# bytedance/DeepSolid

Hardware: AMD Instinct MI355X
Metric: local-energy evals/sec (higher is better)
Workload: dtype f64; 1 GPU; bcc_li 24 e- (12,12), total_energy primal (E_kin forward-Laplacian + Ewald), default detnet ((256,32),)*3, 8 dets; batch_per_gpu=4096, global_batch=4096, parallelism=walker-dp1

## Files before the change

### deepsolid_amd/_lib.py

```python
import ctypes as C
import os

_HERE = os.path.dirname(os.path.abspath(__file__))
LIB_PATH = os.environ.get('DEEPSOLID_HIP_LIB') or os.path.join(_HERE, 'libdeepsolid_hip.so')

DS_MAX_LAYERS = 8
DS_MAX_SYM = 6
_PD = C.POINTER(C.c_double)


class SystemDesc(C.Structure):
    _fields_ = [
        ('dtype', C.c_int32), ('n_up', C.c_int32), ('n_dn', C.c_int32), ('n_atoms_prim', C.c_int32),
        ('prim_atoms', _PD), ('prim_a', C.c_double * 9), ('sim_a', C.c_double * 9), ('n_sym', C.c_int32),
        ('prim_AV', C.c_double * (DS_MAX_SYM * 3)), ('prim_BV', C.c_double * (DS_MAX_SYM * 3)),
        ('sim_AV', C.c_double * (DS_MAX_SYM * 3)), ('sim_BV', C.c_double * (DS_MAX_SYM * 3)),
        ('n_layers', C.c_int32), ('hidden_single', C.c_int32 * DS_MAX_LAYERS),
        ('hidden_double', C.c_int32 * DS_MAX_LAYERS), ('n_det', C.c_int32), ('distance_type', C.c_int32),
        ('envelope_type', C.c_int32), ('full_det', C.c_int32), ('use_last_layer', C.c_int32),
        ('bias_orbitals', C.c_int32), ('klist_up', _PD), ('klist_dn', _PD),
        ('n_atoms_sim', C.c_int32), ('sim_atoms', _PD), ('sim_charges', _PD), ('dist_mode', C.c_int32),
        ('n_g', C.c_int32), ('gpoints', _PD), ('gweight', _PD), ('ion_exp_re', _PD), ('ion_exp_im', _PD),
        ('ewald_alpha', C.c_double), ('ee_const', C.c_double), ('ei_const', C.c_double), ('ii_total', C.c_double),
    ]
# ... 25 lines not shown
        ('a', C.c_double * 9), ('n_atoms', C.c_int32), ('atoms', _PD), ('atom_species', _PI), ('n_species', C.c_int32),
        ('n_l', _PI), ('r_cut_loc', _PD), ('r_cut_nl', _PD), ('term_offset', _PI), ('term_n', _PI), ('term_zeta', _PD),
        ('term_c', _PD), ('n_quad', C.c_int32),
    ]


_VP = C.c_void_p


def _dmc_step_sig(n_lead, n_noise, n_out, ecp):
    step = [C.c_int64, C.c_int] + [C.c_double] * 5 + [C.c_int, C.c_int, C.c_uint64, C.c_uint64]
    return (C.c_int, [_VP] * n_lead + step + [_VP] * n_noise + ([C.c_int64] if ecp else []) + [C.c_int] + [_VP] * n_out +
            ([C.POINTER(C.c_int)] if ecp else []) + [_VP, C.c_int64, _VP])


SIGNATURES = {
    'ds_device_widths': (C.c_int, [C.POINTER(C.c_int32), C.POINTER(C.c_int32), C.c_int32, C.c_int32, C.c_int32, C.c_int32,
                                   C.POINTER(C.c_int32), C.POINTER(C.c_int32), C.POINTER(C.c_int32), C.POINTER(C.c_int32)]),
    'ds_system_create': (C.c_int, [C.POINTER(SystemDesc), C.POINTER(_VP)]),
    'ds_system_destroy': (None, [_VP]),
    'ds_last_error': (C.c_char_p, []),
    'ds_param_count': (C.c_int64, [_VP]),
    'ds_int8_layers': (C.c_int, [_VP]),
    'ds_param_layout': (C.c_int, [_VP, C.POINTER(ParamBlock), C.c_int]),
    'ds_workspace_bytes': (C.c_int64, [_VP, C.c_int64]),
    'ds_logpsi': (C.c_int, [_VP, _VP, _VP, C.c_int64, _VP, _VP, _VP, C.c_int64, _VP]),
    'ds_logpsi_grad': (C.c_int, [_VP, _VP, _VP, C.c_int64, _VP, _VP, _VP, _VP, C.c_int64, _VP]),
    'ds_vjp_workspace_bytes': (C.c_int64, [_VP, C.c_int64]),
    'ds_logpsi_vjp': (C.c_int, [_VP, _VP, _VP, C.c_int64, _VP, _VP, _VP, _VP, _VP, C.c_int64, _VP]),
    'ds_pretrain_workspace_bytes': (C.c_int64, [_VP, C.c_int64]),
    'ds_pretrain_loss_vjp': (C.c_int, [_VP, _VP, _VP, C.c_int64, _VP, _VP, _VP, _VP, _VP, C.c_int64, _VP]),
    'ds_kfac_block_count': (C.c_int, [_VP]),
    'ds_kfac_layout': (C.c_int, [_VP, C.POINTER(KfacBlock), C.c_int]),
    'ds_kfac_workspace_bytes': (C.c_int64, [_VP, C.c_int64]),
    'ds_kfac_factors': (C.c_int, [_VP, _VP, _VP, C.c_int64, _VP, _VP, _VP, C.c_int64, _VP]),
    'ds_kfac_step_workspace_bytes': (C.c_int64, [_VP]),
    'ds_kfac_inverses': (C.c_int, [_VP, _VP, C.c_double, C.c_double, _VP, _VP, C.c_int64, _VP]),
    'ds_kfac_precondition': (C.c_int, [_VP, _VP, _VP, _VP, _VP, _VP, C.c_int64, _VP]),
    'ds_kfac_inverses_sized_workspace_bytes': (C.c_int64, [C.c_int, C.POINTER(C.c_int32), C.POINTER(C.c_int32)]),
    'ds_kfac_inverses_sized': (C.c_int, [C.c_int, C.c_int, C.POINTER(C.c_int32), C.POINTER(C.c_int32), C.POINTER(C.c_int32), _VP,
                                        C.c_double, C.c_double, _VP, _VP, C.c_int64, _VP]),
    'ds_jacobian_workspace_bytes': (C.c_int64, [_VP, C.c_int64]),
    'ds_logpsi_jacobian': (C.c_int, [_VP, _VP, _VP, C.c_int64, _VP, C.c_int64, _VP, _VP, _VP, C.c_int64, _VP]),
    'ds_minsr_gram_workspace_bytes': (C.c_int64, [C.c_int64, C.c_int64]),
    'ds_minsr_gram': (C.c_int, [C.c_int, _VP, C.c_int64, C.c_int64, C.c_int64, _VP, _VP, C.c_int64, _VP]),
    'ds_minsr_matvec_workspace_bytes': (C.c_int64, [C.c_int, C.c_int64, C.c_int64]),
# ... 96 lines not shown
```

### deepsolid_amd/csrc/ds_api.hip

```cpp
#include <cstdarg>

#include "ds_host.h"
#include "ds_tiles.h"

namespace ds {
#define DS_DECL(p) const TileOps<double>* tile_ops_f64_p##p(int); const TileOps<float>* tile_ops_f32_p##p(int);
DS_DECL(0) DS_DECL(1) DS_DECL(2) DS_DECL(3) DS_DECL(4)
#undef DS_DECL
template <> const TileOps<double>* tile_ops<double>(int st) {
    const TileOps<double>* (*parts[])(int) = {tile_ops_f64_p0, tile_ops_f64_p1, tile_ops_f64_p2, tile_ops_f64_p3, tile_ops_f64_p4};
    for (auto f : parts)
        if (const TileOps<double>* o = f(st)) return o;
    return nullptr;
}
template <> const TileOps<float>* tile_ops<float>(int st) {
    const TileOps<float>* (*parts[])(int) = {tile_ops_f32_p0, tile_ops_f32_p1, tile_ops_f32_p2, tile_ops_f32_p3, tile_ops_f32_p4};
    for (auto f : parts)
        if (const TileOps<float>* o = f(st)) return o;
    return nullptr;
}
}

namespace ds {
namespace host {
// ... 318 lines not shown
        for (int l = 0; l <= s->sd.n_layers; ++l) h1max = std::max(h1max, s->sd.h1[l]);
        if (hipMalloc(&s->lr_w0t, (size_t)h1max * 64 * sizeof(double)) != hipSuccess) {
            ds_system_destroy(s);
            return fail("hipMalloc of the low-rank layer's weight table failed");
        }
    }
    {
        hipDeviceProp_t prop;
        int devid = 0;
        if (hipGetDevice(&devid) == hipSuccess && hipGetDeviceProperties(&prop, devid) == hipSuccess && prop.multiProcessorCount > 0)
            s->n_cu = prop.multiProcessorCount;
    }
    if (hipMalloc((void**)&s->clk_dev, 1024 * sizeof(unsigned long long)) != hipSuccess ||
        hipMemset(s->clk_dev, 0, 1024 * sizeof(unsigned long long)) != hipSuccess) {
        ds_system_destroy(s);
        return fail("hipMalloc of the clock-probe counters failed");
    }
    s->det_valu = getenv("DS_DET_VALU") != nullptr;
    if (const char* e = getenv("DS_VAL_NB")) { const int v = atoi(e); s->val_nb = (v == 1 || v == 2 || v == 4) ? v : 0; }
    s->no_lu_wave = getenv("DS_NO_LU_WAVE") != nullptr;
    s->use_lr = getenv("DS_NO_LOWRANK") == nullptr;
    s->use_pm_skip = getenv("DS_NO_PM_SKIP") == nullptr;
    s->use_pair_expand = getenv("DS_NO_PAIR_EXPAND") == nullptr;
    s->use_g4 = getenv("DS_NO_G4") == nullptr;
    s->use_i8 = getenv("DS_I8") != nullptr && getenv("DS_NO_I8") == nullptr;
    s->use_ldsb = getenv("DS_NO_LDSB") == nullptr;
    s->use_pair_fuse = getenv("DS_NO_PAIR_FUSE") == nullptr;
    s->use_i8_val = getenv("DS_NO_I8_VAL") == nullptr;
    for (int l = 0; l < DS_MAX_LAYERS; ++l) s->i8_prepped[l] = ~(uint64_t)0;
    if (const char* e = getenv("DS_I8_VAL_MIN_TILES")) s->val_i8_min_tiles = atoll(e);
    if (const char* e = getenv("DS_DBG")) s->dbg = atoi(e);
    s->use_wide = getenv("DS_NO_WIDE") == nullptr;
    s->wide_all = getenv("DS_WIDE_ALL") != nullptr;
    {
        const size_t bytes = i8_planes_bytes(s);
        if (bytes && hipMalloc(&s->i8_wp, bytes) != hipSuccess) {
            ds_system_destroy(s);
            return fail("hipMalloc of the int8 layer's weight planes failed");
        }
    }
    if (const char* e = getenv("DS_CHUNK_WALKERS")) s->chunk_cap = std::min<int64_t>(65535, std::max<int64_t>(1, atol(e)));
    *out = s;
    return 0;
}

void ds_system_destroy(ds_system* s) {
// ... 110 lines not shown
```

### deepsolid_amd/csrc/ds_chain.hip

```cpp
#include "ds_host.h"
#include "ds_tiles.h"

namespace ds {
namespace host {

template <typename T> inline unsigned m2_split(int K2, int N) {
    unsigned z = 1;
    while (z < 8 && K2 % (2 * z) == 0 && (size_t)(K2 / z) * 5 * N * sizeof(T) > 8192) z *= 2;
    return z;
}

enum Stop { STOP_NONE = 0, STOP_G0, STOP_G1, STOP_G2, STOP_G3, STOP_H2_0, STOP_H2_1, STOP_H2_2, STOP_MEAN0, STOP_Q,
            STOP_MOUT, STOP_MINV, STOP_DETS, STOP_TR };

template <typename T> struct DumpReq { int stop; T* out; int64_t cap; int64_t written; };

template <typename T>
int copy_out(DumpReq<T>* dr, const T* src, size_t n, hipStream_t st) {
    size_t m = std::min<size_t>(n, (size_t)dr->cap);
    HIP_OK(hipMemcpyAsync(dr->out, src, m * sizeof(T), hipMemcpyDeviceToDevice, st));
    dr->written = (int64_t)m;
    return 0;
}

enum class LayerKind {
    Dense,
    DenseRes,
    L0Stats,
    L0Epi9Means,
    LowRank1,
    Int8
};
struct PairPlan {
    bool res, res_sep;
    bool expand;
    bool write_out;
    unsigned xz; int EW, NW; size_t xlds;
};
struct LayerPlan {
    LayerKind kind;
    bool res_sep;
    bool wide;
    bool pm_mask;
    bool pm_unwritten;
    int prof_kind;
    PairPlan pair;
};
enum class OrbKind { Orb3, Wide, Ldsb, Gemm };
template <typename T> struct ChainPlan {
    const ds::TileOps<T>* to;
    bool lr_on;
    int lr_nc;
    int g4;
    LayerPlan layer[DS_MAX_LAYERS];
    OrbKind orb[2];
    int count(LayerKind k, int n_layers) const {
        int n = 0;
        for (int l = 0; l < n_layers; ++l) n += layer[l].kind == k ? 1 : 0;
        return n;
    }
};

template <typename T>
int plan_chain(const ds_system* s, bool dump, ChainPlan<T>* p) {
    const ds::SysDev<double>& S = s->sd;
    const ds::TileOps<T>* to = p->to = ds::tile_ops<T>(S.P / 16);
    if (!to) return fail("no kernel instance for %d slot tiles (N = %d electrons)", S.P / 16, S.N);
    const int ST = to->ST;
    const bool wide = s->use_wide && to->gemm_wide != nullptr;
    auto gemm_wide = [&](int epi) { return wide && (s->wide_all || ds::gemm_wide_faster<T>(epi)); };
    const int K0loc = S.h1[0] + S.nch * S.h2[0], K0sh = S.nch * S.h1[0];
    p->lr_nc = std::max(2, (K0loc + K0sh + 4 + 15) / 16);
    p->lr_on = !dump && s->use_lr && S.n_layers >= 2 && !s->res1[0] && p->lr_nc <= 4 && S.h1[1] % 16 == 0 && (S.nch * S.h2[1]) % 4 == 0 &&
               3 * (K0loc + K0sh + 4) <= S.h1[1] && p->lr_nc * S.h1[1] < (S.h1[1] - K0loc - K0sh - 4) * ST;
    const int used = S.D - 16 * (ST - 1);
    p->g4 = !s->use_g4 ? 0 : (ST == 5 && used > 8 && used <= 12) ? 3 : (ST == 10 && used <= 4) ? 1 : 0;
    for (int l = 0; l < S.n_layers; ++l) {
        const int Kh = S.h1[l], K2 = S.h2[l], Nout = S.h1[l + 1], Kloc = Kh + S.nch * K2;
        LayerPlan& lp = p->layer[l];
        lp = LayerPlan{};
        if (Nout % 64 || Nout > 1024) return fail("hidden_single must be a multiple of 64 and <= 1024 (got %d)", Nout);
        if (l < S.n_double) {
            PairPlan& pp = lp.pair;
            const int K2o = S.h2[l + 1];
            if (K2o != 32 && K2o != 16) return fail("hidden_double must be 16 or 32 (got %d)", K2o);
            if (K2 % 4) return fail("pair-stream width %d is not a multiple of 4", K2);
            pp.res_sep = s->res2[l] && l == 0;
            pp.res = s->res2[l] && !pp.res_sep;
            pp.xz = (!pp.res && K2o == 32) ? 2 : 1;
            pp.write_out = l + 1 < S.n_double || s->use_last;
            pp.EW = (pp.write_out && S.N % 16 == 8 && pp.xz == 2) ? 2 : 1;
            pp.NW = (pp.EW * S.N + 15) / 16;
            pp.xlds = ((size_t)(K2o / pp.xz) * 5 * pp.EW * S.N + (size_t)pp.EW * S.nch * (K2o / pp.xz) * 5) * sizeof(T);
            pp.expand = !dump && s->use_pair_expand && !pp.res_sep && l + 1 < S.n_layers && pp.NW <= 8 && pp.xlds <= 150 * 1024;
        }
        const bool res = s->res1[l];
        lp.res_sep = res && l == 0 && (Kloc % 16 != 0 || S.nf * S.A != Nout);
        if (res && !lp.res_sep && Kloc % 16) return fail("residual layer with K = %d: the GEMM's operand ring needs K %% 16 == 0", Kloc);
        if (p->lr_on && l == 1) {
            lp.kind = LayerKind::LowRank1;
            lp.wide = wide && (s->wide_all || ds::lr_wide_faster<T>(p->lr_nc));
        } else if (p->lr_on && l == 0) {
            const bool one_kernel = to->layer0_stats && ds::layer0_stats_instance(ST, K0loc / 4);
            lp.kind = one_kernel ? LayerKind::L0Stats : LayerKind::L0Epi9Means;
            lp.wide = !one_kernel && gemm_wide(9);
        } else if (int8_energy_layer(s, l)) {
            lp.kind = LayerKind::Int8;
        } else if (res && !lp.res_sep) {
            lp.kind = LayerKind::DenseRes;
            lp.wide = gemm_wide(2);
        } else {
            lp.kind = LayerKind::Dense;
            lp.wide = gemm_wide(1);
        }
        lp.prof_kind = l == 0 ? DS_PROF_SINGLE_FIRST : (lp.kind == LayerKind::LowRank1 ? DS_PROF_SINGLE_LR : DS_PROF_SINGLE_HIDDEN);
        lp.pm_mask = s->use_pm_skip && (l == 0 || (lp.kind == LayerKind::DenseRes && Kh % 16 == 0 && K2 % 16 == 0));
        lp.pm_unwritten = !dump && l >= 1 && !lp.wide &&
// ... 39 lines not shown
    }
    if (stop == STOP_MEAN0) return copy_out(dr, c.MEAN[0], (size_t)S.nch * S.h1[0] * S.P * Bc, st);
    if (stop == STOP_H2_0) return copy_out(dr, c.H2[0], (size_t)S.h2[0] * 5 * S.NP * Bc, st);
    if (stop == STOP_Q) return copy_out(dr, c.Q, L.Q * Bc, st);
    int gi = 0, hi = 0;
    for (int l = 0; l < S.n_layers; ++l) {
        const LayerPlan& lp = plan.layer[l];
        const int Kh = S.h1[l], K2 = S.h2[l], Nout = S.h1[l + 1];
        if (!(l > 0 && plan.layer[l - 1].pair.expand)) {
            ProfScope ps(s, DS_PROF_M2_EXPAND, st);
            const bool xl = lr_on && l == 0;
            hipLaunchKernelGGL((ds::k_m2_expand<T>), dim3(S.N, (unsigned)Bc, m2_split<T>(K2, S.N)), dim3(256), (size_t)(K2 * 5 * S.N + S.nch * K2 * 5) / m2_split<T>(K2, S.N) * sizeof(T), st, S,
                               c.H2[hi], K2, xl ? c.XL : c.G[gi], Kh, xl ? K0loc : S.ldk, lp.pm_unwritten ? 1 : 0);
        }
        if (stop == STOP_G0 + l) return copy_out(dr, c.G[gi], L.G * Bc, st);
        if (l < S.n_double) {
            const PairPlan& pp = lp.pair;
            const int K2o = S.h2[l + 1];
            const T* W2 = blk(s->i_w2[l]); const T* b2 = blk(s->i_b2[l]);
            ProfScope ps(s, DS_PROF_TWO_LAYER, st);
            if (pp.expand) {
#define DS_TWOX(NT2, RES) hipLaunchKernelGGL((ds::k_two_layer_expand<T, NT2, RES>), dim3(S.N / pp.EW, (unsigned)Bc, pp.xz), dim3(64 * pp.NW), pp.xlds, st, S, c.H2[hi], K2, W2, b2, \
                                             pp.write_out ? c.H2[hi ^ 1] : (T*)nullptr, c.G[gi ^ 1], S.h1[l + 1], S.ldk, plan.layer[l + 1].pm_unwritten ? 1 : 0, pp.EW)
                if (K2o == 32 && pp.res) DS_TWOX(2, true);
                else if (pp.res) DS_TWOX(1, true);
                else DS_TWOX(1, false);
#undef DS_TWOX
            } else {
                const dim3 grid((S.NP / 16 + 3) / 4, (unsigned)Bc);
#define DS_TWO(NT2, RES) hipLaunchKernelGGL((ds::k_two_layer<T, NT2, RES, false>), grid, dim3(256), 0, st, S, c.H2[hi], K2, W2, b2, c.H2[hi ^ 1])
                if (K2o == 32) { if (pp.res) DS_TWO(2, true); else DS_TWO(2, false); }
                else { if (pp.res) DS_TWO(1, true); else DS_TWO(1, false); }
#undef DS_TWO
            }
            if (pp.res_sep)
                launch_pair_res_add<T>(dim3((unsigned)(((size_t)K2o * 5 * S.NP + 255) / 256), (unsigned)Bc), st, c.H2[hi], K2, c.H2[hi ^ 1], K2o, S.nf, S.NP);
        }
        const int Kloc = Kh + S.nch * K2, Ksh = S.nch * Kh;
        {
            dim3 block; unsigned gz;
            gemm_geom(Nout, NB, &block, &gz, ST);
            dim3 wblock; unsigned wgz;
            gemm_geom(Nout, 4, &wblock, &wgz, 6);
            const size_t gws = (size_t)S.N * S.ldk * S.P, gts = (size_t)S.ldk * S.P;
            const bool lr1 = lp.kind == LayerKind::LowRank1;
            T* Sl = lr1 ? c.ZB + (size_t)Bc * S.h1[1] * S.P : c.ZB;
            {
                ProfScope ps(s, DS_PROF_SHARED_TERM, st);
                if (l == 0 || lr1) {
// ... 39 lines not shown
                                   (size_t)S.N * K0loc * S.P, (size_t)K0loc * S.P, blk(s->i_wloc[0]), K0loc, c.ZB, Nout, S.P, c.YO, c.MEAN[1]);
                break;
            }
            case LayerKind::Int8: {
                launch_layer_i8(s, l, false, (const double*)blk(s->i_wloc[l]), Kloc, Nout, (const double*)c.G[gi], gts, (const double*)Sl,
                                (double*)c.G[gi ^ 1], (int)(Bc * S.N), st);
                break;
            }
            case LayerKind::DenseRes:
                ga.oe.dbg = s->dbg & 3;
                ga.oe.g4 = plan.g4;
                if (l > 0 && s->prof_on && (s->prof_only < 0 || s->prof_only == DS_PROF_SINGLE_HIDDEN)) { ga.oe.clk = s->clk_dev; ga.oe.dbg = s->dbg; }
                layer_gemm(2, ga);
                break;
            case LayerKind::Dense:
                layer_gemm(1, ga);
                if (lp.res_sep)
                    launch_layer_res_add<T>(dim3(S.N, (unsigned)Bc), st, Xin, xws, xts, c.G[gi ^ 1], gws, gts, S.nf * S.A, Nout, S.P);
                break;
            }
        }
        gi ^= 1;
        if (l < S.n_double) {
            hi ^= 1;
            if (stop == STOP_H2_1 + l) return copy_out(dr, c.H2[hi], (size_t)S.h2[l + 1] * 5 * S.NP * Bc, st);
        }
    }
    if (stop == STOP_G0 + S.n_layers) return copy_out(dr, c.G[gi], L.G * Bc, st);
    const int Kl = S.h1[S.n_layers], K2l = S.h2[S.n_layers];
    if (s->use_last) {
        ProfScope ps(s, DS_PROF_M2_EXPAND, st);
        hipLaunchKernelGGL((ds::k_m2_expand<T>), dim3(S.N, (unsigned)Bc, m2_split<T>(K2l, S.N)), dim3(256), (size_t)(K2l * 5 * S.N + S.nch * K2l * 5) / m2_split<T>(K2l, S.N) * sizeof(T), st, S,
                           c.H2[hi], K2l, c.G[gi], Kl, S.ldk, 0);
    }
    for (int sp = 0; sp < S.nch; ++sp) {
        const int ns = sp == 0 ? S.n_up : S.n_dn, i0 = sp == 0 ? 0 : S.n_up, OC = S.ocols[sp];
        const int Korb = Kl + (s->use_last ? S.nch * K2l : 0);
        dim3 block; unsigned gz;
        gemm_geom(OC, NB, &block, &gz, ST);
        if (s->use_last) {
            ProfScope ps(s, DS_PROF_SHARED_TERM, st);
            to->shared_term(dim3(1, (unsigned)Bc, gz), block, 2 * 16 * S.P * sizeof(T), st, S, c.G[gi], blk(s->i_wsh_orb[sp]), Kl, c.ZB, OC, S.P,
                            (const T*)nullptr, 0);
        }
        ProfScope ps(s, DS_PROF_ORBITAL, st);
        const int ch = S.mat_ch[sp];
        ds::OrbEpi<T> oe{c.Q, c.MOUT, L.MOUT, L.mout_off[ch], S.N, i0, S.nparam[sp], S.nparam_max, S.norb[sp], S.det_n[ch],
// ... 110 lines not shown
    const ds::SysDev<T>& S = dev<T>(s);
    size_t sh = ds::ewald_lds_bytes(S);
    hipLaunchKernelGGL((ds::k_ewald<T>), dim3((unsigned)B), dim3(256), sh, st, S, (const T*)x, (T*)out);
}

template <typename T>
int64_t debug_stage_impl(ds_system* s, const void* params, const void* x, int64_t B, int stop, void* out, int64_t out_elems, void* ws,
                         int64_t ws_bytes, hipStream_t st) {
    DumpReq<T> dr{stop, (T*)out, out_elems, 0};
    const int rc = run_chain<T>(s, (const T*)params, (const T*)x, B, arena_of<T>(ws, ws_bytes), st, nullptr, nullptr, nullptr, &dr);
    return rc ? -1 : dr.written;
}

int logpsi_grad_forward(ds_system* s, const void* params, const void* x, int64_t B, void* out_logabs, void* out_phase, void* out_grad,
                        void* ws, int64_t ws_bytes, hipStream_t st) {
    return DS_BY_DTYPE(s->dtype, logpsi_grad_impl, s, params, x, B, out_logabs, out_phase, out_grad, ws, ws_bytes, st);
}

int int8_energy_layers(const ds_system* s, bool dump) {
    ChainPlan<double> plan;
    return plan_chain<double>(s, dump, &plan) == 0 ? plan.count(LayerKind::Int8, s->sd.n_layers) : 0;
}

template <typename T> void launch_pair_res_add(dim3 grid, hipStream_t st, const T* Hin, int Kin, T* Hout, int Kout, int n_res, int NP) {
    hipLaunchKernelGGL((ds::k_pair_res_add<T>), grid, dim3(256), 0, st, Hin, Kin, Hout, Kout, n_res, NP);
}

template <typename T>
void launch_layer_res_add(dim3 grid, hipStream_t st, const T* Xin, size_t x_ws, size_t x_ts, T* Gout, size_t g_ws, size_t g_ts, int n_res,
                          int Nout, int P) {
    hipLaunchKernelGGL((ds::k_layer_res_add<T>), grid, dim3(256), 0, st, Xin, x_ws, x_ts, Gout, g_ws, g_ts, n_res, Nout, P);
}

#define DS_INST(T)                                                                                      \
    template void launch_pair_res_add<T>(dim3, hipStream_t, const T*, int, T*, int, int, int);          \
    template void launch_layer_res_add<T>(dim3, hipStream_t, const T*, size_t, size_t, T*, size_t, size_t, int, int, int);
DS_INST(double) DS_INST(float)
#undef DS_INST

}
}

using namespace ds::host;

extern "C" {

int ds_int8_layers(const ds_system* s) {
    if (!s) return -1;
    return int8_energy_layers(s, false);
}

int ds_local_energy(ds_system* s, const void* params, const void* x, int64_t B, void* out_ke, void* out_ewald, void* out_logabs,
                    void* out_phase, void* ws, int64_t ws_bytes, void* stream) {
    if (s) ++s->call_seq;
    if (!s || !params || !x || !ws) return fail("null argument");
    if (B <= 0) return 0;
    hipStream_t st = (hipStream_t)stream;
    return DS_BY_DTYPE(s->dtype, local_energy_impl, s, params, x, B, out_ke, out_ewald, out_logabs, out_phase, ws, ws_bytes, st);
}

int ds_logpsi_grad(ds_system* s, const void* params, const void* x, int64_t B, void* out_logabs, void* out_phase, void* out_grad,
                   void* ws, int64_t ws_bytes, void* stream) {
    if (s) ++s->call_seq;
    if (!s || !params || !x || !ws || !out_grad) return fail("null argument");
    if (B <= 0) return 0;
    hipStream_t st = (hipStream_t)stream;
    return logpsi_grad_forward(s, params, x, B, out_logabs, out_phase, out_grad, ws, ws_bytes, st);
}

int ds_ewald(ds_system* s, const void* x, int64_t B, void* out, void* stream) {
    if (!s || !x || !out) return fail("null argument");
    if (B <= 0) return 0;
// ... 27 lines not shown
```

### deepsolid_amd/csrc/ds_host.h

```cpp
#pragma once
#include "ds_base.h"
#include "ds_value.h"

namespace ds {
namespace host {

template <typename I> inline I rup(I x, int m) { return (x + m - 1) / m * m; }

template <typename T> struct Arena {
    T* base = nullptr;
    size_t cap = SIZE_MAX, used = 0;
    bool ok = true;
    T* take(size_t n) { T* p = base ? base + used : nullptr; used += n; ok = ok && used <= cap; return p; }
    void align(size_t k) { take((k - used % k) % k); }
    template <typename F> void part(T* buf, size_t n, F&& carve) { Arena a{buf, n}; carve(a); ok = ok && a.ok; }
};
template <typename T> Arena<T> arena_of(void* ws, int64_t ws_bytes) { return Arena<T>{(T*)ws, (size_t)std::max<int64_t>(ws_bytes, 0) / sizeof(T)}; }
template <typename F> size_t measure(F&& layout) { Arena<double> a; layout(a); return a.used; }

struct PassSize { size_t fixed, per_group; };
inline int64_t groups_per_pass(int64_t B, int64_t esz, const PassSize& z, int64_t budget) {
    const int64_t groups = std::min<int64_t>((std::max<int64_t>(B, 1) + ds::PV - 1) / ds::PV, 64);
    return std::max<int64_t>(1, std::min<int64_t>(groups, budget / ((int64_t)z.per_group * esz)));
}
// ... 16 lines not shown
}

struct ds_system {
    ds_system_desc d;
    int dtype;
    ds::SysDev<double> sd;
    ds::SysDev<float> sf;
    void* blob64 = nullptr;
    void* blob32 = nullptr;
    std::vector<ds_param_block> blocks;
    int64_t nparams = 0;
    ds::host::WsLayout ws;
    ds::host::WsLayout wsv;
    std::vector<int> i_wloc, i_wsh, i_b, i_w2, i_b2, i_worb, i_wsh_orb, i_borb, i_pi, i_sg;
    bool use_last = false;
    int32_t ref_single[DS_MAX_LAYERS] = {0}, ref_double[DS_MAX_LAYERS] = {0};
    bool res1[DS_MAX_LAYERS] = {false}, res2[DS_MAX_LAYERS] = {false};
    bool no_lu_wave = false;
    int val_nb = 0;
    bool det_valu = false;
    int64_t chunk_cap = 4096;
    bool use_g4 = true;
    bool use_pair_expand = true;
    bool use_pm_skip = true;
    bool use_lr = true;
    void* lr_w0t = nullptr;
    int64_t val_i8_min_tiles = 512;
    bool use_i8_val = true;
    bool use_pair_fuse = true;
    bool use_ldsb = true;
    bool use_i8 = false;
    void* i8_wp = nullptr;
    uint64_t call_seq = 0;
    uint64_t i8_prepped[DS_MAX_LAYERS];
    int n_cu = 256;
    bool use_wide = true;
    bool wide_all = false;
    int dbg = 0;
    bool prof_on = false;
    int prof_only = -1;
    std::vector<std::pair<hipEvent_t, hipEvent_t>> prof_ev[DS_PROF_KINDS];
    std::vector<hipEvent_t> prof_pool;
    unsigned long long* clk_dev = nullptr;
    bool prof_failed = false;
};

// ... 175 lines not shown
```

### deepsolid_amd/csrc/ds_kernels.h

```cpp
#pragma once
#include "ds_device.h"

namespace ds {

#define DS_MAXL 8

template <typename T> struct SysDev {
    int N, n_up, n_dn, A, L, K, nch;
    int D, P, NP;
    int n_layers, n_double;
    int h1[DS_MAXL + 1];
    int h2[DS_MAXL + 1];
    int ldk;
    int full_det, env_type, bias_orb;
    int dist_type, nf;
    int norb[2];
    int n_detch;
    int det_n[2];
    int mat_ch[2], row_off[2];
    int nparam[2];
    int nparam_max;
    int ocols[2];
    const T *prim_a, *prim_ainv, *sim_a, *sim_ainv, *prim_AV, *prim_BV, *sim_AV, *sim_BV, *atoms;
    const T* klist[2];
// ... 191 lines not shown
template <typename T>
__global__ void __launch_bounds__(256) k_layer_res_add(const T* __restrict__ Xin, size_t x_ws, size_t x_ts, T* __restrict__ Gout, size_t g_ws,
                                                       size_t g_ts, int n_res, int Nout, int P) {
    const T* xi = Xin + (size_t)blockIdx.y * x_ws + (size_t)blockIdx.x * x_ts;
    T* go = Gout + (size_t)blockIdx.y * g_ws + (size_t)blockIdx.x * g_ts;
    const T rs2 = T(0.70710678118654752440);
    for (int idx = threadIdx.x; idx < Nout * P; idx += blockDim.x) {
        const T r = idx < n_res * P ? xi[idx] : T(0);
        go[idx] = (r + go[idx]) * rs2;
    }
}

template <typename T>
__global__ void __launch_bounds__(256) k_pair_res_add(const T* __restrict__ Hin, int Kin, T* __restrict__ Hout, int Kout, int n_res, int NP) {
    const size_t idx = (size_t)blockIdx.x * blockDim.x + threadIdx.x;
    if (idx >= (size_t)Kout * 5 * NP) return;
    const T* hi = Hin + (size_t)blockIdx.y * Kin * 5 * NP;
    T* ho = Hout + (size_t)blockIdx.y * Kout * 5 * NP;
    const T r = idx < (size_t)n_res * 5 * NP ? hi[idx] : T(0);
    ho[idx] = (r + ho[idx]) * T(0.70710678118654752440);
}

constexpr int PM_SLOTS = 3;
template <typename T, int NT2, bool RES, bool VAL>
__global__ void __launch_bounds__(256, ((RES && !VAL && sizeof(T) == 8 && NT2 == 2) ? 2 : 3)) k_two_layer(SysDev<T> S, const T* __restrict__ Hin, int Kin, const T* __restrict__ W,
                                                   const T* __restrict__ bias, T* __restrict__ Hout, T* __restrict__ PARTM = nullptr) {
    typedef typename Acc4<T>::type acc_t;
    const int w = blockIdx.y, wave = threadIdx.x >> 6, lane = threadIdx.x & 63;
    const int pt = blockIdx.x * 4 + wave, NP = S.NP, Kout = 16 * NT2;
    if (pt * 16 >= NP) return;
    const int lr = lane & 15, lq = lane >> 4;
    const T* Hw = Hin + (size_t)w * Kin * 5 * NP + pt * 16 + lr;
    acc_t acc[NT2][5];
#pragma unroll
    for (int a = 0; a < NT2; ++a)
#pragma unroll
        for (int c = 0; c < 5; ++c) acc[a][c] = acc_t{0, 0, 0, 0};
    constexpr bool KEEP = RES && !VAL && sizeof(T) == 8;
    T bk[KEEP ? 4 * NT2 : 1][5];
    if constexpr (KEEP) {
#pragma unroll
        for (int ks = 0; ks < 4 * NT2; ++ks)
#pragma unroll
            for (int c = 0; c < 5; ++c) bk[ks][c] = Hw[(size_t)((4 * ks + lq) * 5 + c) * NP];
#pragma unroll
        for (int ks = 0; ks < 4 * NT2; ++ks) {
// ... 16 lines not shown
        for (int a = 0; a < NT2; ++a)
#pragma unroll
            for (int c = 0; c < 5; ++c) acc[a][c] = mfma16(av[a], bv[c], acc[a][c]);
    }
    const T rs2 = T(0.70710678118654752440);
    T* Ho = Hout + (size_t)w * Kout * 5 * NP + pt * 16 + lr;
    __shared__ T pm_stage[VAL ? 4 * PM_SLOTS * 16 * NT2 * 5 : 1];
    T* pm_lds = pm_stage + (VAL ? wave * (PM_SLOTS * Kout * 5) : 0);
    bool pm_valid = false, pm_last = false;
    int pm_slot = 0;
    if (VAL && PARTM) {
        const int N = S.N, nch = S.nch;
        auto seg_of = [&](int p) { const int e = p / N, j = p - e * N; return p < N * N ? e * nch + (nch > 1 && j >= S.n_up ? 1 : 0) : -1; };
        const int p = pt * 16 + lr, sg = seg_of(p);
        pm_valid = sg >= 0;
        pm_slot = sg - seg_of(pt * 16);
        pm_last = pm_valid && (lr == 15 || seg_of(p + 1) != sg);
    }
#pragma unroll
    for (int a = 0; a < NT2; ++a)
#pragma unroll
        for (int r = 0; r < 4; ++r) {
            const int n = 16 * a + acc_row<T>(lane, r);
            const T z0 = acc[a][0][r] + bias[n];
            const T y = ds_tanh(z0), d1 = 1 - y * y, d2 = -2 * y * d1;
            const T z1 = acc[a][1][r], z2 = acc[a][2][r], z3 = acc[a][3][r], z4 = acc[a][4][r];
            T o[5] = {y, d1 * z1, d1 * z2, d1 * z3, d1 * z4 + d2 * 2 * (z1 * z1 + z2 * z2 + z3 * z3)};
            if (VAL) {
                o[1] = ds_tanh(z1 + bias[n]); o[2] = ds_tanh(z2 + bias[n]); o[3] = ds_tanh(z3 + bias[n]); o[4] = ds_tanh(z4 + bias[n]);
            }
#pragma unroll
            for (int c = 0; c < 5; ++c) {
                T v = o[c];
                if (RES) v = ((KEEP ? bk[KEEP ? 4 * a + r : 0][c] : Hw[(size_t)(n * 5 + c) * NP]) + v) * rs2;
                if (Hout) Ho[(size_t)(n * 5 + c) * NP] = v;
                if (VAL && PARTM) {
                    const T pre = row16_prefix(pm_valid ? v : T(0));
                    if (pm_last) pm_lds[(pm_slot * Kout + n) * 5 + c] = pre;
                }
            }
        }
    if (VAL && PARTM) {
        __builtin_amdgcn_fence(__ATOMIC_ACQ_REL, "wavefront");
        __builtin_amdgcn_wave_barrier();
        T* pm = PARTM + ((size_t)w * (NP / 16) + pt) * (PM_SLOTS * Kout * 5);
        for (int i = lane; i < PM_SLOTS * Kout * 5; i += 64) pm[i] = pm_lds[i];
    }
}

template <typename T, int NT2, bool RES>
__global__ void __launch_bounds__(512) k_two_layer_expand(SysDev<T> S, const T* __restrict__ Hin, int Kin, const T* __restrict__ W,
                                                          const T* __restrict__ bias, T* __restrict__ Hout, T* __restrict__ G, int row0,
                                                          int ldg, int skip, int EW) {
    typedef typename Acc4<T>::type acc_t;
    extern __shared__ __attribute__((aligned(16))) char smem_raw[];
    const int w = blockIdx.y, wave = threadIdx.x >> 6, lane = threadIdx.x & 63, tid = threadIdx.x, nt = blockDim.x;
    const int N = S.N, NP = S.NP, P = S.P, Kout = 16 * NT2, e0 = blockIdx.x * EW, PW = EW * N;
    const int KT = Kout * gridDim.z, n0 = Kout * blockIdx.z;
    const int lr = lane & 15, lq = lane >> 4;
    const bool valid = wave * 16 + lr < PW;
    const int pl = valid ? wave * 16 + lr : PW - 1;
    const T* Hw = Hin + (size_t)w * Kin * 5 * NP + e0 * N + pl;
    T* hs = reinterpret_cast<T*>(smem_raw);
    T* sums = hs + Kout * 5 * PW;
    acc_t acc[NT2][5];
#pragma unroll
    for (int a = 0; a < NT2; ++a)
#pragma unroll
        for (int c = 0; c < 5; ++c) acc[a][c] = acc_t{0, 0, 0, 0};
    constexpr bool KEEP = RES && sizeof(T) == 8;
    T bk[KEEP ? 4 * NT2 : 1][5];
    if constexpr (KEEP) {
#pragma unroll
        for (int ks = 0; ks < 4 * NT2; ++ks)
#pragma unroll
            for (int c = 0; c < 5; ++c) bk[ks][c] = Hw[(size_t)((4 * ks + lq) * 5 + c) * NP];
#pragma unroll
        for (int ks = 0; ks < 4 * NT2; ++ks) {
            T av[NT2];
#pragma unroll
            for (int a = 0; a < NT2; ++a) av[a] = W[(size_t)(4 * ks + lq) * KT + n0 + 16 * a + lr];
#pragma unroll
            for (int a = 0; a < NT2; ++a)
#pragma unroll
                for (int c = 0; c < 5; ++c) acc[a][c] = mfma16(av[a], bk[ks][c], acc[a][c]);
        }
    } else
    for (int ks = 0; ks < Kin / 4; ++ks) {
        T av[NT2], bv[5];
#pragma unroll
        for (int a = 0; a < NT2; ++a) av[a] = W[(size_t)(4 * ks + lq) * KT + n0 + 16 * a + lr];
#pragma unroll
        for (int c = 0; c < 5; ++c) bv[c] = Hw[(size_t)((4 * ks + lq) * 5 + c) * NP];
#pragma unroll
        for (int a = 0; a < NT2; ++a)
#pragma unroll
            for (int c = 0; c < 5; ++c) acc[a][c] = mfma16(av[a], bv[c], acc[a][c]);
    }
    const T rs2 = T(0.70710678118654752440);
    T* Ho = (Hout && valid) ? Hout + ((size_t)w * KT + n0) * 5 * NP + e0 * N + pl : nullptr;
#pragma unroll
    for (int a = 0; a < NT2; ++a)
#pragma unroll
        for (int r = 0; r < 4; ++r) {
            const int n = 16 * a + acc_row<T>(lane, r);
            const T z0 = acc[a][0][r] + bias[n0 + n];
            const T y = ds_tanh(z0), d1 = 1 - y * y, d2 = -2 * y * d1;
            const T z1 = acc[a][1][r], z2 = acc[a][2][r], z3 = acc[a][3][r], z4 = acc[a][4][r];
            const T o[5] = {y, d1 * z1, d1 * z2, d1 * z3, d1 * z4 + d2 * 2 * (z1 * z1 + z2 * z2 + z3 * z3)};
#pragma unroll
            for (int c = 0; c < 5; ++c) {
                T v = o[c];
                if (RES) v = ((KEEP ? bk[KEEP ? 4 * a + r : 0][c] : Hw[(size_t)((n0 + n) * 5 + c) * NP]) + v) * rs2;
                if (Ho) Ho[(size_t)(n * 5 + c) * NP] = v;
                if (valid) hs[(n * 5 + c) * PW + pl] = v;
            }
        }
    __syncthreads();
    const int nch = S.nch;
    for (int idx = tid; idx < EW * nch * Kout * 5; idx += nt) {
        const int kc = idx % (5 * Kout), es = idx / (5 * Kout), s = es % nch, el = es / nch;
        const int j0 = s == 0 ? 0 : S.n_up, ns = s == 0 ? S.n_up : S.n_dn;
        T v = 0;
        for (int j = j0; j < j0 + ns; ++j) v += hs[kc * PW + el * N + j];
        sums[idx] = v / T(ns);
    }
    __syncthreads();
    typedef T vec4 __attribute__((ext_vector_type(4)));
    const int QP = P / 4;
    for (int idx = tid; idx < EW * nch * Kout * QP; idx += nt) {
        const int row = idx / QP, sq = idx - row * QP, k = row % Kout, es = row / Kout, s = es % nch, el = es / nch, e = e0 + el;
        const int j0 = s == 0 ? 0 : S.n_up, ns = s == 0 ? S.n_up : S.n_dn;
        if (skip) {
            const int t = sq >> 2, lo = (2 + 3 * j0) >> 4, hi = (4 + 3 * (j0 + ns - 1)) >> 4;
            if (!(t == 0 || t == ((2 + 3 * e) >> 4) || t == ((4 + 3 * e) >> 4) || (t >= lo && t <= hi))) continue;
        }
        const T inv = T(1) / T(ns);
        const T* sm = sums + (es * Kout + k) * 5;
        vec4 v;
#pragma unroll
        for (int u = 0; u < 4; ++u) {
            const int slot = 4 * sq + u;
            T x = 0;
            if (slot == 0) x = sm[0];
            else if (slot == 1) x = sm[4];
            else if (slot < S.D) {
                const int j = (slot - 2) / 3, c = (slot - 2) - 3 * j;
                if (j == e) x = -sm[1 + c];
                else if (j >= j0 && j < j0 + ns) x = hs[(k * 5 + 1 + c) * PW + el * N + j] * inv;
            }
            v[u] = x;
        }
        *reinterpret_cast<vec4*>(G + ((size_t)(w * N + e) * ldg + row0 + s * KT + n0 + k) * P + 4 * sq) = v;
    }
}

template <typename T>
__global__ void __launch_bounds__(256) k_m2_combine_val(SysDev<T> S, const T* __restrict__ PARTM, int K2, T* __restrict__ G, int row0, int RC) {
    constexpr int PV_ = 80;
    extern __shared__ __attribute__((aligned(16))) char smem_raw[];
    T* out = reinterpret_cast<T*>(smem_raw);
    const int e = blockIdx.x, g = blockIdx.y, N = S.N, nt = S.NP / 16, nch = S.nch;
    const int r0 = blockIdx.z * RC, sp = r0 / K2, k0 = r0 - sp * K2;
    const size_t blk = (size_t)PM_SLOTS * K2 * 5;
    const int a = e * N + (sp == 0 ? 0 : S.n_up), ns = sp == 0 ? S.n_up : S.n_dn, b = a + ns;
    const int seg = e * nch + sp;
    for (int idx = threadIdx.x; idx < RC * PV_; idx += blockDim.x) {
        const int cc = idx % 5, kk = (idx / 5) % RC, w5 = idx / (5 * RC), k = k0 + kk;
        const T* pw = PARTM + ((size_t)g * (PV_ / 5) + w5) * nt * blk;
        T v = 0;
        for (int pt = a / 16; pt <= (b - 1) / 16; ++pt) {
            const int p0 = pt * 16, e0 = p0 / N, j0 = p0 - e0 * N, seg0 = e0 * nch + (nch > 1 && j0 >= S.n_up ? 1 : 0);
            const int q = seg - seg0;
            v += pw[(size_t)pt * blk + ((size_t)q * K2 + k) * 5 + cc] - (q > 0 ? pw[(size_t)pt * blk + ((size_t)(q - 1) * K2 + k) * 5 + cc] : T(0));
        }
        out[kk * PV_ + w5 * 5 + cc] = v / T(ns);
// ... 950 lines not shown
```

### deepsolid_amd/device.py

```python
import ctypes as C
import re
from typing import NamedTuple

import numpy as np
import torch

from . import _lib
from .params import ParamMap

_DTYPES = {torch.float64: 0, torch.float32: 1}


def _pd(a):
    return a.ctypes.data_as(C.POINTER(C.c_double))


def _ptr(t):
    return C.c_void_p(t.data_ptr()) if t is not None else C.c_void_p(0)


def _stream():
    return C.c_void_p(torch.cuda.current_stream().cuda_stream)


# ... 793 lines not shown
        return dict(e_loc=energy[:, 0], e_nl=torch.complex(energy[:, 1], energy[:, 2]), pairs=pairs if want_pairs else None,
                    rotations=rot, pair_capacity=cap,
                    ratios=torch.view_as_complex(ratios)[:int(pairs.sum()) * ecp.n_quad] if want_ratios else None)

    def energy_stats(self, ke, ew):
        out = torch.empty(8, dtype=torch.float64, device=self.device)
        _lib.check(self.lib.ds_energy_stats(self.handle, _ptr(ke), _ptr(ew), ke.shape[0], _ptr(out), _stream()), 'ds_energy_stats')
        return out

    def profile(self, on=True, only=None):
        mode = 0 if not on else (1 if only is None else 2 + _lib.PROF_KINDS.index(only))
        _lib.check(self.lib.ds_profile_enable(self.handle, mode), 'ds_profile_enable')

    def profile_read(self):
        n = len(_lib.PROF_KINDS)
        ms = (C.c_double * n)()
        cnt = (C.c_int64 * n)()
        _lib.check(self.lib.ds_profile_read(self.handle, ms, cnt), 'ds_profile_read')
        return {k: (float(ms[i]), int(cnt[i])) for i, k in enumerate(_lib.PROF_KINDS)}

    def int8_layers(self):
        return int(self.lib.ds_int8_layers(self.handle))

    def profile_clock(self):
        cyc, ticks = C.c_double(0), C.c_double(0)
        _lib.check(self.lib.ds_profile_read_clock(self.handle, C.byref(cyc), C.byref(ticks)), 'ds_profile_read_clock')
        return cyc.value, ticks.value, (cyc.value / ticks.value * 0.1 if ticks.value > 0 else None)

    def debug_stage(self, params, x, stage, n_elems):
        x = self._check_x(x)
        p = self.pack_params(params)
        ws = self.workspace(x.shape[0])
        out = torch.zeros(int(n_elems), dtype=self.dtype, device=self.device)
        n = self.lib.ds_debug_stage(self.handle, _ptr(p), _ptr(x), x.shape[0], stage.encode(), _ptr(out), out.numel(),
                                    _ptr(ws), ws.numel(), _stream())
        if n < 0:
            raise RuntimeError(f'ds_debug_stage({stage}): {self.lib.ds_last_error().decode()}')
        return out[:n]


def observable_sums(recvec, x, q_int, pol_direction):
    _require_gpu()
    if not x.is_cuda:
        raise RuntimeError('observable_sums: walkers must live on the ROCm device (no CPU path)')
    if x.dtype not in _DTYPES:
        raise TypeError(f'observable_sums: walkers must be float64 or float32, got {x.dtype}')
# ... 238 lines not shown
```

### include/deepsolid_hip.h

```cpp
#ifndef DEEPSOLID_HIP_H
#define DEEPSOLID_HIP_H

#include <stddef.h>
#include <stdint.h>

#ifdef __cplusplus
extern "C" {
#endif

#define DS_MAX_LAYERS 8
#define DS_MAX_SYM 6

typedef struct ds_system ds_system;

typedef struct ds_system_desc {
    int32_t dtype;
    int32_t n_up, n_dn;
    int32_t n_atoms_prim;
    const double* prim_atoms;
    double prim_a[9];
    double sim_a[9];
    int32_t n_sym;
    double prim_AV[DS_MAX_SYM * 3], prim_BV[DS_MAX_SYM * 3];
    double sim_AV[DS_MAX_SYM * 3], sim_BV[DS_MAX_SYM * 3];
// ... 18 lines not shown
    const double* ion_exp_re;
    const double* ion_exp_im;
    double ewald_alpha;
    double ee_const;
    double ei_const;
    double ii_total;
} ds_system_desc;

typedef struct ds_param_block {
    int64_t offset;
    int32_t rows, cols;
} ds_param_block;

int ds_device_widths(const int32_t* hidden_single, const int32_t* hidden_double, int32_t n_layers, int32_t n_in_single,
                     int32_t n_in_double, int32_t n_double, int32_t* dev_single, int32_t* dev_double, int32_t* res_single,
                     int32_t* res_double);

int ds_system_create(const ds_system_desc* desc, ds_system** out);
void ds_system_destroy(ds_system* sys);
const char* ds_last_error(void);

int ds_int8_layers(const ds_system* sys);

int64_t ds_param_count(const ds_system* sys);
int ds_param_layout(const ds_system* sys, ds_param_block* blocks, int max_blocks);

int64_t ds_workspace_bytes(const ds_system* sys, int64_t B);

int ds_logpsi(ds_system* sys, const void* params, const void* x, int64_t B,
              void* out_logabs, void* out_phase, void* ws, int64_t ws_bytes, void* stream);

int ds_logpsi_grad(ds_system* sys, const void* params, const void* x, int64_t B,
                   void* out_logabs, void* out_phase, void* out_grad, void* ws, int64_t ws_bytes, void* stream);

int64_t ds_vjp_workspace_bytes(const ds_system* sys, int64_t B);
int ds_logpsi_vjp(ds_system* sys, const void* params, const void* x, int64_t B, const void* cot, void* grad,
                  void* out_logabs, void* out_phase, void* ws, int64_t ws_bytes, void* stream);

int64_t ds_pretrain_workspace_bytes(const ds_system* sys, int64_t B);
int ds_pretrain_loss_vjp(ds_system* sys, const void* params, const void* x, int64_t B, const void* target_up,
                         const void* target_dn, void* out_loss, void* grad, void* ws, int64_t ws_bytes, void* stream);

typedef struct ds_kfac_block {
    int32_t kind, index;
    int32_t n_param_blocks;
    int32_t param_blocks[3];
// ... 216 lines not shown
```

Before: 67580 local-energy evals/s.

## Recompute narrow preceding pair layer inside residual expand kernel instead of storing it

When a float64 residual pair layer follows a narrow (≤8 wide) non-residual expanded pair layer, the previous layer no longer writes its pair-stream output. The next expand kernel recomputes that layer's tanh jet from its input via MFMA and keeps the result in registers, which removes a global write and read of the pair activations at the cost of redundant matmul work. The G-scatter loop in the expand kernel is also restructured so per-slot indexing is hoisted out of the row loop. A query API reports how many layers use the recompute path, and an env var disables it.

```diff
diff --git a/deepsolid_amd/_lib.py b/deepsolid_amd/_lib.py
--- a/deepsolid_amd/_lib.py
+++ b/deepsolid_amd/_lib.py
@@ -71,6 +71,7 @@
     'ds_last_error': (C.c_char_p, []),
     'ds_param_count': (C.c_int64, [_VP]),
     'ds_int8_layers': (C.c_int, [_VP]),
+    'ds_pair_recompute_layers': (C.c_int, [_VP, C.c_int]),
     'ds_param_layout': (C.c_int, [_VP, C.POINTER(ParamBlock), C.c_int]),
     'ds_workspace_bytes': (C.c_int64, [_VP, C.c_int64]),
     'ds_logpsi': (C.c_int, [_VP, _VP, _VP, C.c_int64, _VP, _VP, _VP, C.c_int64, _VP]),
diff --git a/deepsolid_amd/csrc/ds_api.hip b/deepsolid_amd/csrc/ds_api.hip
--- a/deepsolid_amd/csrc/ds_api.hip
+++ b/deepsolid_amd/csrc/ds_api.hip
@@ -364,6 +364,7 @@
     s->use_lr = getenv("DS_NO_LOWRANK") == nullptr;
     s->use_pm_skip = getenv("DS_NO_PM_SKIP") == nullptr;
     s->use_pair_expand = getenv("DS_NO_PAIR_EXPAND") == nullptr;
+    s->use_pair_recompute = getenv("DS_NO_PAIR_RECOMPUTE") == nullptr;
     s->use_g4 = getenv("DS_NO_G4") == nullptr;
     s->use_i8 = getenv("DS_I8") != nullptr && getenv("DS_NO_I8") == nullptr;
     s->use_ldsb = getenv("DS_NO_LDSB") == nullptr;
diff --git a/deepsolid_amd/csrc/ds_chain.hip b/deepsolid_amd/csrc/ds_chain.hip
--- a/deepsolid_amd/csrc/ds_chain.hip
+++ b/deepsolid_amd/csrc/ds_chain.hip
@@ -36,6 +36,7 @@
     bool expand;
     bool write_out;
     unsigned xz; int EW, NW; size_t xlds;
+    bool recompute_prev;
 };
 struct LayerPlan {
     LayerKind kind;
@@ -75,6 +76,12 @@
                3 * (K0loc + K0sh + 4) <= S.h1[1] && p->lr_nc * S.h1[1] < (S.h1[1] - K0loc - K0sh - 4) * ST;
     const int used = S.D - 16 * (ST - 1);
     p->g4 = !s->use_g4 ? 0 : (ST == 5 && used > 8 && used <= 12) ? 3 : (ST == 10 && used <= 4) ? 1 : 0;
+    auto pair_geom = [&](PairPlan& pp, int K2o) {
+        pp.xz = (!pp.res && K2o == 32) ? 2 : 1;
+        pp.EW = (pp.write_out && S.N % 16 == 8 && pp.xz == 2) ? 2 : 1;
+        pp.NW = (pp.EW * S.N + 15) / 16;
+        pp.xlds = ((size_t)(K2o / pp.xz) * 5 * pp.EW * S.N + (size_t)pp.EW * S.nch * (K2o / pp.xz) * 5) * sizeof(T);
+    };
     for (int l = 0; l < S.n_layers; ++l) {
         const int Kh = S.h1[l], K2 = S.h2[l], Nout = S.h1[l + 1], Kloc = Kh + S.nch * K2;
         LayerPlan& lp = p->layer[l];
@@ -87,12 +94,18 @@
             if (K2 % 4) return fail("pair-stream width %d is not a multiple of 4", K2);
             pp.res_sep = s->res2[l] && l == 0;
             pp.res = s->res2[l] && !pp.res_sep;
-            pp.xz = (!pp.res && K2o == 32) ? 2 : 1;
             pp.write_out = l + 1 < S.n_double || s->use_last;
-            pp.EW = (pp.write_out && S.N % 16 == 8 && pp.xz == 2) ? 2 : 1;
-            pp.NW = (pp.EW * S.N + 15) / 16;
-            pp.xlds = ((size_t)(K2o / pp.xz) * 5 * pp.EW * S.N + (size_t)pp.EW * S.nch * (K2o / pp.xz) * 5) * sizeof(T);
+            pair_geom(pp, K2o);
             pp.expand = !dump && s->use_pair_expand && !pp.res_sep && l + 1 < S.n_layers && pp.NW <= 8 && pp.xlds <= 150 * 1024;
+            if (l >= 1) {
+                PairPlan& prev = p->layer[l - 1].pair;
+                pp.recompute_prev = sizeof(T) == 8 && !dump && s->use_pair_recompute && pp.res && pp.expand && S.h2[l - 1] <= 8 &&
+                                    !prev.res && !prev.res_sep && prev.expand;
+                if (pp.recompute_prev) {
+                    prev.write_out = false;
+                    pair_geom(prev, K2);
+                }
+            }
         }
         const bool res = s->res1[l];
         lp.res_sep = res && l == 0 && (Kloc % 16 != 0 || S.nf * S.A != Nout);
@@ -178,9 +191,15 @@
             if (pp.expand) {
 #define DS_TWOX(NT2, RES) hipLaunchKernelGGL((ds::k_two_layer_expand<T, NT2, RES>), dim3(S.N / pp.EW, (unsigned)Bc, pp.xz), dim3(64 * pp.NW), pp.xlds, st, S, c.H2[hi], K2, W2, b2, \
                                              pp.write_out ? c.H2[hi ^ 1] : (T*)nullptr, c.G[gi ^ 1], S.h1[l + 1], S.ldk, plan.layer[l + 1].pm_unwritten ? 1 : 0, pp.EW)
-                if (K2o == 32 && pp.res) DS_TWOX(2, true);
+#define DS_TWOXP(NT2) hipLaunchKernelGGL((ds::k_two_layer_expand<T, NT2, true, true>), dim3(S.N / pp.EW, (unsigned)Bc, pp.xz), dim3(64 * pp.NW), pp.xlds, st, S, c.H2[hi ^ 1], S.h2[l - 1], W2, b2, \
+                                         pp.write_out ? c.H2[hi] : (T*)nullptr, c.G[gi ^ 1], S.h1[l + 1], S.ldk, plan.layer[l + 1].pm_unwritten ? 1 : 0, pp.EW,               \
+                                         blk(s->i_w2[l - 1]), blk(s->i_b2[l - 1]))
+                if (pp.recompute_prev) {
+                    if constexpr (sizeof(T) == 8) { if (K2o == 32) DS_TWOXP(2); else DS_TWOXP(1); }
+                } else if (K2o == 32 && pp.res) DS_TWOX(2, true);
                 else if (pp.res) DS_TWOX(1, true);
                 else DS_TWOX(1, false);
+#undef DS_TWOXP
 #undef DS_TWOX
             } else {
                 const dim3 grid((S.NP / 16 + 3) / 4, (unsigned)Bc);
@@ -266,7 +285,7 @@
         }
         gi ^= 1;
         if (l < S.n_double) {
-            hi ^= 1;
+            if (!lp.pair.recompute_prev) hi ^= 1;
             if (stop == STOP_H2_1 + l) return copy_out(dr, c.H2[hi], (size_t)S.h2[l + 1] * 5 * S.NP * Bc, st);
         }
     }
@@ -423,6 +442,14 @@
     return plan_chain<double>(s, dump, &plan) == 0 ? plan.count(LayerKind::Int8, s->sd.n_layers) : 0;
 }
 
+template <typename T> int pair_recompute_count(const ds_system* s, bool dump) {
+    ChainPlan<T> plan;
+    if (plan_chain<T>(s, dump, &plan)) return 0;
+    int n = 0;
+    for (int l = 0; l < s->sd.n_double && l < s->sd.n_layers; ++l) n += plan.layer[l].pair.recompute_prev ? 1 : 0;
+    return n;
+}
+
 template <typename T> void launch_pair_res_add(dim3 grid, hipStream_t st, const T* Hin, int Kin, T* Hout, int Kout, int n_res, int NP) {
     hipLaunchKernelGGL((ds::k_pair_res_add<T>), grid, dim3(256), 0, st, Hin, Kin, Hout, Kout, n_res, NP);
 }
@@ -449,6 +476,11 @@
 int ds_int8_layers(const ds_system* s) {
     if (!s) return -1;
     return int8_energy_layers(s, false);
+}
+
+int ds_pair_recompute_layers(const ds_system* s, int dump) {
+    if (!s) return -1;
+    return s->dtype == 0 ? pair_recompute_count<double>(s, dump != 0) : pair_recompute_count<float>(s, dump != 0);
 }
 
 int ds_local_energy(ds_system* s, const void* params, const void* x, int64_t B, void* out_ke, void* out_ewald, void* out_logabs,
diff --git a/deepsolid_amd/csrc/ds_host.h b/deepsolid_amd/csrc/ds_host.h
--- a/deepsolid_amd/csrc/ds_host.h
+++ b/deepsolid_amd/csrc/ds_host.h
@@ -62,6 +62,7 @@
     int64_t chunk_cap = 4096;
     bool use_g4 = true;
     bool use_pair_expand = true;
+    bool use_pair_recompute = true;
     bool use_pm_skip = true;
     bool use_lr = true;
     void* lr_w0t = nullptr;
diff --git a/deepsolid_amd/csrc/ds_kernels.h b/deepsolid_amd/csrc/ds_kernels.h
--- a/deepsolid_amd/csrc/ds_kernels.h
+++ b/deepsolid_amd/csrc/ds_kernels.h
@@ -237,6 +237,13 @@
 }
 
 constexpr int PM_SLOTS = 3;
+template <typename T>
+__device__ __forceinline__ void pair_tanh_jet(T z0, T z1, T z2, T z3, T z4, T (&o)[5]) {
+    const T y = ds_tanh(z0), d1 = 1 - y * y, d2 = -2 * y * d1;
+    o[0] = y; o[1] = d1 * z1; o[2] = d1 * z2; o[3] = d1 * z3;
+    o[4] = d1 * z4 + d2 * 2 * (z1 * z1 + z2 * z2 + z3 * z3);
+}
+__device__ __forceinline__ double as_loaded(double x) { asm("" : "+v"(x)); return x; }
 template <typename T, int NT2, bool RES, bool VAL>
 __global__ void __launch_bounds__(256, ((RES && !VAL && sizeof(T) == 8 && NT2 == 2) ? 2 : 3)) k_two_layer(SysDev<T> S, const T* __restrict__ Hin, int Kin, const T* __restrict__ W,
                                                    const T* __restrict__ bias, T* __restrict__ Hout, T* __restrict__ PARTM = nullptr) {
@@ -299,10 +306,9 @@
 #pragma unroll
         for (int r = 0; r < 4; ++r) {
             const int n = 16 * a + acc_row<T>(lane, r);
-            const T z0 = acc[a][0][r] + bias[n];
-            const T y = ds_tanh(z0), d1 = 1 - y * y, d2 = -2 * y * d1;
             const T z1 = acc[a][1][r], z2 = acc[a][2][r], z3 = acc[a][3][r], z4 = acc[a][4][r];
-            T o[5] = {y, d1 * z1, d1 * z2, d1 * z3, d1 * z4 + d2 * 2 * (z1 * z1 + z2 * z2 + z3 * z3)};
+            T o[5];
+            pair_tanh_jet(acc[a][0][r] + bias[n], z1, z2, z3, z4, o);
             if (VAL) {
                 o[1] = ds_tanh(z1 + bias[n]); o[2] = ds_tanh(z2 + bias[n]); o[3] = ds_tanh(z3 + bias[n]); o[4] = ds_tanh(z4 + bias[n]);
             }
@@ -325,10 +331,11 @@
     }
 }
 
-template <typename T, int NT2, bool RES>
+template <typename T, int NT2, bool RES, bool PREV = false>
 __global__ void __launch_bounds__(512) k_two_layer_expand(SysDev<T> S, const T* __restrict__ Hin, int Kin, const T* __restrict__ W,
                                                           const T* __restrict__ bias, T* __restrict__ Hout, T* __restrict__ G, int row0,
-                                                          int ldg, int skip, int EW) {
+                                                          int ldg, int skip, int EW, const T* __restrict__ W0 = nullptr,
+                                                          const T* __restrict__ b0 = nullptr) {
     typedef typename Acc4<T>::type acc_t;
     extern __shared__ __attribute__((aligned(16))) char smem_raw[];
     const int w = blockIdx.y, wave = threadIdx.x >> 6, lane = threadIdx.x & 63, tid = threadIdx.x, nt = blockDim.x;
@@ -346,12 +353,40 @@
 #pragma unroll
         for (int c = 0; c < 5; ++c) acc[a][c] = acc_t{0, 0, 0, 0};
     constexpr bool KEEP = RES && sizeof(T) == 8;
+    static_assert(!PREV || KEEP, "the layer in front is recomputed into the kept operands of a float64 residual layer");
     T bk[KEEP ? 4 * NT2 : 1][5];
     if constexpr (KEEP) {
-#pragma unroll
-        for (int ks = 0; ks < 4 * NT2; ++ks)
-#pragma unroll
-            for (int c = 0; c < 5; ++c) bk[ks][c] = Hw[(size_t)((4 * ks + lq) * 5 + c) * NP];
+        if constexpr (PREV) {
+            for (int ks = 0; ks < Kin / 4; ++ks) {
+                T av[NT2], bv[5];
+#pragma unroll
+                for (int a = 0; a < NT2; ++a) av[a] = W0[(size_t)(4 * ks + lq) * Kout + 16 * a + lr];
+#pragma unroll
+                for (int c = 0; c < 5; ++c) bv[c] = Hw[(size_t)((4 * ks + lq) * 5 + c) * NP];
+#pragma unroll
+                for (int a = 0; a < NT2; ++a)
+#pragma unroll
+                    for (int c = 0; c < 5; ++c) acc[a][c] = mfma16(av[a], bv[c], acc[a][c]);
+            }
+#pragma unroll
+            for (int a = 0; a < NT2; ++a)
+#pragma unroll
+                for (int r = 0; r < 4; ++r) {
+                    T o[5];
+                    pair_tanh_jet(acc[a][0][r] + b0[16 * a + acc_row<T>(lane, r)], acc[a][1][r], acc[a][2][r], acc[a][3][r], acc[a][4][r], o);
+#pragma unroll
+                    for (int c = 0; c < 5; ++c) bk[4 * a + r][c] = as_loaded(o[c]);
+                }
+#pragma unroll
+            for (int a = 0; a < NT2; ++a)
+#pragma unroll
+                for (int c = 0; c < 5; ++c) acc[a][c] = acc_t{0, 0, 0, 0};
+        } else {
+#pragma unroll
+            for (int ks = 0; ks < 4 * NT2; ++ks)
+#pragma unroll
+                for (int c = 0; c < 5; ++c) bk[ks][c] = Hw[(size_t)((4 * ks + lq) * 5 + c) * NP];
+        }
 #pragma unroll
         for (int ks = 0; ks < 4 * NT2; ++ks) {
             T av[NT2];
@@ -381,10 +416,8 @@
 #pragma unroll
         for (int r = 0; r < 4; ++r) {
             const int n = 16 * a + acc_row<T>(lane, r);
-            const T z0 = acc[a][0][r] + bias[n0 + n];
-            const T y = ds_tanh(z0), d1 = 1 - y * y, d2 = -2 * y * d1;
-            const T z1 = acc[a][1][r], z2 = acc[a][2][r], z3 = acc[a][3][r], z4 = acc[a][4][r];
-            const T o[5] = {y, d1 * z1, d1 * z2, d1 * z3, d1 * z4 + d2 * 2 * (z1 * z1 + z2 * z2 + z3 * z3)};
+            T o[5];
+            pair_tanh_jet(acc[a][0][r] + bias[n0 + n], acc[a][1][r], acc[a][2][r], acc[a][3][r], acc[a][4][r], o);
 #pragma unroll
             for (int c = 0; c < 5; ++c) {
                 T v = o[c];
@@ -404,31 +437,39 @@
     }
     __syncthreads();
     typedef T vec4 __attribute__((ext_vector_type(4)));
-    const int QP = P / 4;
-    for (int idx = tid; idx < EW * nch * Kout * QP; idx += nt) {
-        const int row = idx / QP, sq = idx - row * QP, k = row % Kout, es = row / Kout, s = es % nch, el = es / nch, e = e0 + el;
-        const int j0 = s == 0 ? 0 : S.n_up, ns = s == 0 ? S.n_up : S.n_dn;
-        if (skip) {
-            const int t = sq >> 2, lo = (2 + 3 * j0) >> 4, hi = (4 + 3 * (j0 + ns - 1)) >> 4;
-            if (!(t == 0 || t == ((2 + 3 * e) >> 4) || t == ((4 + 3 * e) >> 4) || (t >= lo && t <= hi))) continue;
-        }
-        const T inv = T(1) / T(ns);
-        const T* sm = sums + (es * Kout + k) * 5;
-        vec4 v;
+    const int QP = P / 4, CW = QP < nt ? QP : nt, RPP = nt / CW, rsub = tid / CW;
+    const T inv_s[2] = {T(1) / T(S.n_up), T(1) / T(nch > 1 ? S.n_dn : S.n_up)};
+    if (rsub < RPP)
+    for (int sq = tid - rsub * CW; sq < QP; sq += CW) {
+        int kind[4], smi[4], sj[4], hoff[4];
 #pragma unroll
         for (int u = 0; u < 4; ++u) {
-            const int slot = 4 * sq + u;
-            T x = 0;
-            if (slot == 0) x = sm[0];
-            else if (slot == 1) x = sm[4];
-            else if (slot < S.D) {
-                const int j = (slot - 2) / 3, c = (slot - 2) - 3 * j;
-                if (j == e) x = -sm[1 + c];
-                else if (j >= j0 && j < j0 + ns) x = hs[(k * 5 + 1 + c) * PW + el * N + j] * inv;
-            }
-            v[u] = x;
-        }
-        *reinterpret_cast<vec4*>(G + ((size_t)(w * N + e) * ldg + row0 + s * KT + n0 + k) * P + 4 * sq) = v;
+            const int slot = 4 * sq + u, j = (slot - 2) / 3, c = (slot - 2) - 3 * j;
+            kind[u] = slot < 2 ? 1 : slot < S.D ? 2 : 0;
+            smi[u] = slot == 0 ? 0 : slot == 1 ? 4 : kind[u] == 2 ? 1 + c : 0;
+            sj[u] = kind[u] == 2 ? j : 0;
+            hoff[u] = kind[u] == 2 ? (1 + c) * PW + j : 0;
+        }
+        const int t = sq >> 2;
+        for (int row = rsub; row < EW * nch * Kout; row += RPP) {
+            const int k = row % Kout, es = row / Kout, s = nch > 1 ? es & 1 : 0, el = nch > 1 ? es >> 1 : es, e = e0 + el;
+            const int j0 = s == 0 ? 0 : S.n_up, ns = s == 0 ? S.n_up : S.n_dn;
+            if (skip) {
+                const int lo = (2 + 3 * j0) >> 4, hi = (4 + 3 * (j0 + ns - 1)) >> 4;
+                if (!(t == 0 || t == ((2 + 3 * e) >> 4) || t == ((4 + 3 * e) >> 4) || (t >= lo && t <= hi))) continue;
+            }
+            const T inv = inv_s[s];
+            const T* sm = sums + (es * Kout + k) * 5;
+            const T* hk = hs + k * 5 * PW + el * N;
+            vec4 v;
+#pragma unroll
+            for (int u = 0; u < 4; ++u) {
+                const T m = sm[smi[u]], h = hk[hoff[u]];
+                const bool own = sj[u] == e, partner = sj[u] >= j0 && sj[u] < j0 + ns;
+                v[u] = kind[u] == 2 ? (own ? -m : partner ? h * inv : T(0)) : kind[u] == 1 ? m : T(0);
+            }
+            *reinterpret_cast<vec4*>(G + ((size_t)(w * N + e) * ldg + row0 + s * KT + n0 + k) * P + 4 * sq) = v;
+        }
     }
 }
 
diff --git a/deepsolid_amd/device.py b/deepsolid_amd/device.py
--- a/deepsolid_amd/device.py
+++ b/deepsolid_amd/device.py
@@ -839,6 +839,9 @@
     def int8_layers(self):
         return int(self.lib.ds_int8_layers(self.handle))
 
+    def pair_recompute_layers(self, dump=False):
+        return int(self.lib.ds_pair_recompute_layers(self.handle, 1 if dump else 0))
+
     def profile_clock(self):
         cyc, ticks = C.c_double(0), C.c_double(0)
         _lib.check(self.lib.ds_profile_read_clock(self.handle, C.byref(cyc), C.byref(ticks)), 'ds_profile_read_clock')
diff --git a/include/deepsolid_hip.h b/include/deepsolid_hip.h
--- a/include/deepsolid_hip.h
+++ b/include/deepsolid_hip.h
@@ -64,6 +64,8 @@
 
 int ds_int8_layers(const ds_system* sys);
 
+int ds_pair_recompute_layers(const ds_system* sys, int dump);
+
 int64_t ds_param_count(const ds_system* sys);
 int ds_param_layout(const ds_system* sys, ds_param_block* blocks, int max_blocks);
 
```

Result: faster. 68550 local-energy evals/s (median of 6 runs) (+1.4%).
